# giuspugl/COSMOMAP2

Measured on AMD Instinct MI355X. Metric: TOD samples/s through P^T N^-1 P, higher is better.
Workload: dtype f64

## Files before the change

cosmomap2_amd/csrc/cm2_os_policy.h:

```cpp
#pragma once
#include <cstddef>
#include <cstdint>
#include <vector>

namespace cm2::os {

constexpr int kT = 256;
constexpr int kPts = 32;
constexpr int kHalo = 2048;
constexpr int N = kT * kPts;
constexpr int W = 2 * N;
constexpr int HOP = W - 2 * kHalo;
constexpr int RR = 2;
constexpr int RSLOTS = (kPts - 8) / RR;
constexpr int RLEN = 512 * RSLOTS;
constexpr int NLIST = 2 + RR;
constexpr int PER = 2 * N + HOP;
constexpr int LDSD = N + N / 32;
constexpr int list_off(int l) { return l <= 2 ? l * N : 2 * N + (l - 2) * RLEN; }
constexpr int list_len(int l) { return l < 2 ? N : RLEN; }

struct WinDesc {
    int64_t start, len, lo, hi;
    int32_t blk, pad;
};

inline std::vector<WinDesc> windows(const std::vector<int64_t> &off)
{
    std::vector<WinDesc> wins;
    for (size_t b = 0; b + 1 < off.size(); ++b)
        for (int64_t s0 = off[b]; s0 < off[b + 1]; s0 += HOP)
            wins.push_back({s0, off[b + 1] - s0 < HOP ? off[b + 1] - s0 : HOP, off[b], off[b + 1], (int32_t)b, 0});
    return wins;
}

inline int rmax(int64_t ntiles)
{
    const int64_t bound = ntiles > 0 && ntiles < N ? ntiles : N;
    return (int)((bound + 63) / 64 * 64);
}

constexpr int kTabRows = 8;
inline bool table_fits(int rmax_) { return rmax_ <= kTabRows * kT; }

enum class Builder { sorted, direct, inverse };
struct ListChoice { Builder builder; int mode, rmax; };
inline ListChoice choose_lists(int want_lists, bool build_sort, bool has_tile_off, int64_t ntiles)
{
    const int want = want_lists ? want_lists : (ntiles >= 768 ? 3 : 2);
    const bool direct = !build_sort && has_tile_off && ntiles > 0 && ntiles <= 4096;
    const int r = rmax(ntiles);
    const Builder b = !direct ? Builder::sorted : (want == 3 && table_fits(r) ? Builder::inverse : Builder::direct);
    return {b, b == Builder::inverse ? 3 : (want >= 2 && table_fits(r) ? 2 : 1), r};
}

inline uint32_t descriptor_bytes(int64_t nvalid, bool flat)
{
    return nvalid > 0 && nvalid * 8 < (int64_t)0xFFFFFFF0u && !flat ? (uint32_t)(nvalid * 8) : 0u;
}

inline size_t kernel_lds_bytes(int mode, int rmax_)
{
    return sizeof(double) * (size_t)LDSD + (mode >= 2 ? sizeof(uint32_t) * 2 * (size_t)rmax_ : 0) + 2048;
}

}
```

cosmomap2_amd/csrc/cm2_overlap_save.hip:

```cpp
#include "cm2_os_lists.h"

#include <cstring>
#include <memory>
#include <mutex>

using namespace cm2;

namespace {

constexpr double kCos32[32] = {1.0, 0.9807852804032304, 0.9238795325112867, 0.8314696123025452, 0.7071067811865476, 0.5555702330196022, 0.3826834323650898, 0.19509032201612828, 0.0, -0.19509032201612828, -0.3826834323650898, -0.5555702330196022, -0.7071067811865476, -0.8314696123025452, -0.9238795325112867, -0.9807852804032304, -1.0, -0.9807852804032304, -0.9238795325112867, -0.8314696123025452, -0.7071067811865476, -0.5555702330196022, -0.3826834323650898, -0.19509032201612828, 0.0, 0.19509032201612828, 0.3826834323650898, 0.5555702330196022, 0.7071067811865476, 0.8314696123025452, 0.9238795325112867, 0.9807852804032304};
constexpr double kSin32[32] = {0.0, 0.19509032201612828, 0.3826834323650898, 0.5555702330196022, 0.7071067811865476, 0.8314696123025452, 0.9238795325112867, 0.9807852804032304, 1.0, 0.9807852804032304, 0.9238795325112867, 0.8314696123025452, 0.7071067811865476, 0.5555702330196022, 0.3826834323650898, 0.19509032201612828, 0.0, -0.19509032201612828, -0.3826834323650898, -0.5555702330196022, -0.7071067811865476, -0.8314696123025452, -0.9238795325112867, -0.9807852804032304, -1.0, -0.9807852804032304, -0.9238795325112867, -0.8314696123025452, -0.7071067811865476, -0.5555702330196022, -0.3826834323650898, -0.19509032201612828};

__host__ __device__ constexpr int ilog2(int r) { return r <= 1 ? 0 : 1 + ilog2(r >> 1); }

template <int R>
__host__ __device__ constexpr int brev(int m)
{
    int out = 0;
    for (int b = 0; b < ilog2(R); ++b) out |= ((m >> b) & 1) << (ilog2(R) - 1 - b);
    return out;
}

template <class T> __device__ __forceinline__ T ld_list(const T *p) { return __builtin_nontemporal_load(p); }


#ifndef CM2_OS_TIMING
#define CM2_OS_TIMING 0
#endif
#if CM2_OS_TIMING & 1
#define OS_XF(...) do { } while (0)
#else
#define OS_XF(...) do { __VA_ARGS__; } while (0)
#endif

#ifdef CM2_OS_STAMPS
static unsigned long long *g_os_stamps_host = nullptr;
static unsigned long long *os_stamp_buf()
{
    static unsigned long long *dummy = nullptr;
    if (g_os_stamps_host) return g_os_stamps_host;
    if (!dummy && cm2::dev_malloc(&dummy, sizeof(unsigned long long) * 8 * (1 << 20)) != hipSuccess) abort();
    return dummy;
}
#define OS_STAMP_PARAM , unsigned long long *__restrict__ stamps
#define OS_STAMP_ARG , os_stamp_buf()
#define OS_STAMP(i) (stamps[(int64_t)win * 8 + (i)] = __builtin_amdgcn_s_memtime())
#else
#define OS_STAMP_PARAM
#define OS_STAMP_ARG
#define OS_STAMP(i) do { } while (0)
#endif

template <int L>
__device__ __forceinline__ int reg_base(int t)
{
    if (L == 1) return t + (t >> 5);
    if (L == 2) return (t >> 4) * 264 + (t & 15);
    return 33 * t;
}
template <int L>
__host__ __device__ constexpr int reg_off(int m)
{
    return L == 1 ? 264 * m : (L == 2 ? 4224 * (m >> 4) + 16 * (m & 15) + ((m & 15) >> 1) : m);
}
template <int PERM>
__host__ __device__ constexpr int reg_slot(int m)
{
    return PERM == 32 ? brev<32>(m) : (PERM == 16 ? 16 * (m >> 4) + brev<16>(m & 15) : m);
}

template <int FROM, int TO, int PERM>
__device__ __forceinline__ void reg_exchange(double (&a)[kPts], double *__restrict__ buf, int t)
{
    double *__restrict__ wp = buf + reg_base<FROM>(t);
    const double *__restrict__ rp = buf + reg_base<TO>(t);
#pragma unroll
    for (int m = 0; m < kPts; ++m) wp[reg_off<FROM>(m)] = a[reg_slot<PERM>(m)];
    __syncthreads();
#pragma unroll
    for (int m = 0; m < kPts; ++m) a[m] = rp[reg_off<TO>(m)];
    __syncthreads();
}

template <int R, int OFF>
__device__ __forceinline__ void dft_sub(double (&re)[kPts], double (&im)[kPts])
{
#pragma unroll
    for (int h = R / 2; h >= 1; h >>= 1) {
#pragma unroll
        for (int blk = 0; blk < R; blk += 2 * h) {
#pragma unroll
            for (int i = 0; i < h; ++i) {
                const int a = OFF + blk + i, b = a + h;
                const int tw = i * (32 / (2 * h));
                const double ar = re[a], ai = im[a], br = re[b], bi = im[b];
                re[a] = ar + br;
                im[a] = ai + bi;
                const double dr = ar - br, di = ai - bi;
                if (tw == 0) {
                    re[b] = dr;
                    im[b] = di;
                } else if (tw == 8) {
                    re[b] = di;
                    im[b] = -dr;
                } else {
                    const double c = kCos32[tw], s = kSin32[tw];
                    re[b] = dr * c + di * s;
                    im[b] = di * c - dr * s;
                }
            }
        }
    }
}

template <int R, int OFF>
__device__ __forceinline__ void dit_sub(double (&re)[kPts], double (&im)[kPts])
{
#pragma unroll
    for (int h = 1; h <= R / 2; h <<= 1) {
#pragma unroll
        for (int blk = 0; blk < R; blk += 2 * h) {
#pragma unroll
            for (int i = 0; i < h; ++i) {
                const int a = OFF + blk + i, b = a + h;
                const int tw = i * (32 / (2 * h));
                double tr, ti;
                if (tw == 0) {
                    tr = re[b];
                    ti = im[b];
                } else if (tw == 8) {
                    tr = im[b];
                    ti = -re[b];
                } else {
                    const double c = kCos32[tw], s = kSin32[tw];
                    tr = re[b] * c + im[b] * s;
                    ti = im[b] * c - re[b] * s;
                }
                const double ar = re[a], ai = im[a];
                re[a] = ar + tr;
                im[a] = ai + ti;
                re[b] = ar - tr;
                im[b] = ai - ti;
            }
        }
    }
}

template <int R, int OFF>
__device__ __forceinline__ void reg_fwd(double (&xr)[kPts], double (&xi)[kPts], double2 w1)
{
    dft_sub<R, OFF>(xr, xi);
    double cr = 1.0, ci = 0.0;
#pragma unroll
    for (int m = 1; m < R; ++m) {
        const double nr = cr * w1.x - ci * w1.y;
        ci = cr * w1.y + ci * w1.x;
        cr = nr;
        const int i = OFF + brev<R>(m);
        const double tr = xr[i] * cr - xi[i] * ci;
        xi[i] = xr[i] * ci + xi[i] * cr;
        xr[i] = tr;
    }
}

template <int R, int OFF>
__device__ __forceinline__ void reg_inv(double (&xr)[kPts], double (&xi)[kPts], double2 w1)
{
    double cr = 1.0, ci = 0.0;
#pragma unroll
    for (int m = 1; m < R; ++m) {
        const double nr = cr * w1.x - ci * w1.y;
        ci = cr * w1.y + ci * w1.x;
        cr = nr;
        const int i = OFF + m;
        const double tr = xr[i] * cr + xi[i] * ci;
        xi[i] = xi[i] * cr - xr[i] * ci;
        xr[i] = tr;
    }
    dft_sub<R, OFF>(xi, xr);
}

typedef unsigned int v2u_t __attribute__((ext_vector_type(2)));
template <int E>
__device__ __forceinline__ void q_request(const uint16_t *q, int t, uint32_t (&qq)[E / 2])
{
    asm volatile("" : "+v"(t));
    const v2u_t *p = reinterpret_cast<const v2u_t *>(q) + (E / 4) * 64 * (t >> 6) + (t & 63);
#pragma unroll
    for (int i = 0; i < E / 4; ++i) {
        const v2u_t v = __builtin_nontemporal_load(p + 64 * i);
        qq[2 * i] = v.x;
        qq[2 * i + 1] = v.y;
    }
}
template <int E2>
__device__ __forceinline__ uint32_t q_word(const uint32_t (&qq)[E2], int u) { return (qq[u >> 1] >> (16 * (u & 1))) & 0xFFFFu; }

struct ListArgs {
    const uint32_t *k;
    const uint16_t *q;
    const ListHdr *hdr;
    const uint32_t *tab;
};

__device__ __forceinline__ void tab_dma(const uint32_t *gtab, uint32_t *tab_lds, int rmax, int wave_, int t)
{
    int wave = wave_;
    asm volatile("" : "+s"(wave));
    asm volatile("" : "+v"(t));
    const uint32_t *g = gtab + 64 * wave + (t & 63);
#pragma unroll
    for (int i = 0; i < kTabRows; ++i)
        if (64 * wave + kT * i < rmax)
            __builtin_amdgcn_global_load_lds((const __attribute__((address_space(1))) void *)(g + kT * i),
                                             (__attribute__((address_space(3))) void *)(tab_lds + 64 * wave + kT * i),
                                             4, 0, 0);
}

template <int E, class F>
__device__ __forceinline__ void run_decode(F starts, const uint32_t *__restrict__ tab_lds, int wbase, uint32_t nvalid,
                                           uint32_t s0, uint32_t (&kk)[E])
{
    int rb = wbase;
    asm volatile("" : "+v"(s0));
#pragma unroll
    for (int u = 0; u < E; ++u) {
        const bool flag = starts(u);
        const uint64_t mask = __ballot(flag);
        const int below = __builtin_amdgcn_mbcnt_hi((uint32_t)(mask >> 32),
                                                    __builtin_amdgcn_mbcnt_lo((uint32_t)mask, 0u));
        int r = rb + below + (flag ? 1 : 0);
        rb += __popcll(mask);
        r = r < 0 ? 0 : r;
        const uint32_t s = s0 + 64u * (uint32_t)u;
        const uint32_t a = tab_lds[r] + s;
        kk[u] = s < nvalid ? a : kInvalidSample;
    }
}
template <int E>
__device__ __forceinline__ void rc_decode(const uint32_t (&qq)[E / 2], const uint32_t *__restrict__ tab_lds,
                                          int wbase, uint32_t nvalid, int t, uint32_t (&kk)[E])
{
    run_decode<E>([&](int u) { return (qq[u >> 1] & (0x8000u << (16 * (u & 1)))) != 0u; }, tab_lds, wbase, nvalid,
                  (uint32_t)slot_of<E>(t, 0), kk);
}


template <int E>
__device__ __forceinline__ void idecode(uint32_t fw, const uint32_t *__restrict__ tab_lds, int wbase,
                                        uint32_t nvalid, uint32_t soff, int t, uint32_t (&kk)[E])
{
    run_decode<E>([&](int u) { return ((fw >> u) & 1u) != 0u; }, tab_lds, wbase, nvalid,
                  soff + (uint32_t)slot_of<E>(t, 0), kk);
}

template <int BP>
__device__ __forceinline__ void partner_filter_half(double (&zr)[kPts], double (&zi)[kPts], double *__restrict__ buf,
                                                    double *__restrict__ xbuf, int t, const double2 *__restrict__ ab_own,
                                                    const double2 *__restrict__ ab_blk)
{
    constexpr int H = kPts / 2;
    double *__restrict__ wp = buf + reg_base<3>(t);
    const bool special = t < 8;
    const double2 *__restrict__ ab_prt = ab_blk + (special ? t : 263 - t);
    double2 ca[BP], cb[BP];
    auto request = [&](int m0) {
        int o = m0 * kT;
        asm volatile("" : "+v"(o));
#pragma unroll
        for (int i = 0; i < BP; ++i) {
            ca[i] = ab_own[o + i * kT];
            cb[i] = ab_prt[(kPts - 1) * kT - o - i * kT];
        }
    };
    request(0);
    __builtin_amdgcn_sched_barrier(0);
#pragma unroll
    for (int j = 0; j < H; ++j) {
        wp[H + j] = zr[reg_slot<16>(H + j)];
        wp[j] = zi[reg_slot<16>(H + j)];
    }
    if (special) {
#pragma unroll
        for (int j = 0; j < H; ++j) {
            xbuf[t * H + j] = zr[reg_slot<16>(j)];
            xbuf[(8 + t) * H + j] = zi[reg_slot<16>(j)];
        }
    }
    __syncthreads();
    if (!special) {
        double *__restrict__ pp = buf + 33 * (263 - t) + 31;
#pragma unroll
        for (int m0 = 0; m0 < H; m0 += BP) {
            if (m0 > 0) request(m0);
#pragma unroll
            for (int i0 = 0; i0 < BP; i0 += 4) {
                double pre[4], pim[4];
#pragma unroll
                for (int i = 0; i < 4; ++i) {
                    pre[i] = pp[-(m0 + i0 + i)];
                    pim[i] = pp[-H - (m0 + i0 + i)];
                }
#pragma unroll
                for (int i = 0; i < 4; ++i) {
                    const int m = m0 + i0 + i, sl = reg_slot<16>(m);
                    const double a = ca[i0 + i].x, b = ca[i0 + i].y, ap = cb[i0 + i].x, bp = cb[i0 + i].y;
                    const double nr = a * zr[sl] + b * pim[i];
                    const double ni = a * zi[sl] + b * pre[i];
                    const double qr = ap * pre[i] + bp * zi[sl];
                    const double qi = ap * pim[i] + bp * zr[sl];
                    zr[sl] = nr;
                    zi[sl] = ni;
                    pp[-m] = qr;
                    pp[-H - m] = qi;
                }
            }
            __builtin_amdgcn_sched_barrier(0);
        }
    } else {
        const int tl = t == 0 ? 0 : 8 - t;
        const double *__restrict__ up = buf + 33 * (7 - t) + 47;
#pragma unroll
        for (int m0 = 0; m0 < H; m0 += BP) {
            if (m0 > 0) request(m0);
#pragma unroll
            for (int i = 0; i < BP; ++i) {
                const int m = m0 + i, sl = reg_slot<16>(m);
                const int ms = t == 0 ? (m == 0 ? 0 : H - m) : H - 1 - m;
                const double pre_ = xbuf[tl * H + ms], pim_ = xbuf[(8 + tl) * H + ms];
                const double nr = ca[i].x * zr[sl] + ca[i].y * pim_;
                const double ni = ca[i].x * zi[sl] + ca[i].y * pre_;
                zr[sl] = nr;
                zi[sl] = ni;
                const int mu = kPts - 1 - m, su = reg_slot<16>(mu);
                const double ure = up[-mu], uim = up[-mu - H];
                zr[su] = cb[i].x * wp[mu] + cb[i].y * uim;
                zi[su] = cb[i].x * wp[mu - H] + cb[i].y * ure;
            }
            __builtin_amdgcn_sched_barrier(0);
        }
    }
    __syncthreads();
    if (!special) {
#pragma unroll
        for (int j = 0; j < H; ++j) {
            zr[reg_slot<16>(H + j)] = wp[H + j];
            zi[reg_slot<16>(H + j)] = wp[j];
        }
    }
    __syncthreads();
}

__device__ __forceinline__ void forward_passes(double (&zr)[kPts], double (&zi)[kPts], double *buf, int t,
                                               const double2 *Wtw)
{
    const double2 w_a = Wtw[t];
    const double2 w_b = Wtw[kPts * (t & 15)];
    reg_fwd<kPts, 0>(zr, zi, w_a);
    reg_exchange<1, 2, kPts>(zr, buf, t);
    reg_exchange<1, 2, kPts>(zi, buf, t);
    reg_fwd<16, 0>(zr, zi, w_b);
    reg_fwd<16, 16>(zr, zi, w_b);
    reg_exchange<2, 3, 16>(zr, buf, t);
    reg_exchange<2, 3, 16>(zi, buf, t);
}

__device__ __forceinline__ void inverse_tail(double (&zr)[kPts], double (&zi)[kPts], double *buf, int t, double2 w_bi,
                                             double2 w_ai)
{
    reg_inv<16, 0>(zr, zi, w_bi);
    reg_inv<16, 16>(zr, zi, w_bi);
    reg_exchange<2, 1, 16>(zr, buf, t);
    reg_exchange<2, 1, 16>(zi, buf, t);
    reg_inv<kPts, 0>(zr, zi, w_ai);
}

template <int MODE, bool BUF>
__global__ __launch_bounds__(kT, 2) void k_os_real(
    const WinDesc *__restrict__ wins, int nwin, const double2 *__restrict__ Wtw, const double2 *Wtw_inv,
    const double2 *__restrict__ AB, const uint32_t *__restrict__ lst_k, const uint16_t *__restrict__ lst_q,
    const ListHdr *__restrict__ hdrs, const uint32_t *__restrict__ tabs, int rmax, const double *__restrict__ v,
    double *__restrict__ out, uint32_t nbytes, const IListHdr *__restrict__ ihdrs,
    const uint32_t *__restrict__ iflags OS_STAMP_PARAM)
{
    constexpr int N = os::N, H = kPts / 2;
    constexpr int ER = os::RLEN / kT;
    __amdgpu_buffer_rsrc_t v_rs, o_rs;
    if constexpr (BUF) {
        v_rs = __builtin_amdgcn_make_buffer_rsrc(const_cast<double *>(v), 0, (int)nbytes, 0x00020000);
        o_rs = __builtin_amdgcn_make_buffer_rsrc(out, 0, (int)nbytes, 0x00020000);
    }
    auto gather = [&](uint32_t k) -> double {
        if constexpr (BUF) {
            const v2u_t r = __builtin_amdgcn_raw_buffer_load_b64(v_rs, k * 8u, 0, 0);
            return __builtin_bit_cast(double, r);
        } else {
            return v[k != kInvalidSample ? k : 0u];
        }
    };
    auto keep = [&](uint32_t k, double x) -> double {
        if constexpr (BUF) return x;
        return k != kInvalidSample ? x : 0.0;
    };
    extern __shared__ double buf[];
    uint32_t *__restrict__ tab_lds = reinterpret_cast<uint32_t *>(buf + os::LDSD);
    const int t = threadIdx.x;
    const int per_xcd = (nwin + 7) / 8;
    const int win = (blockIdx.x & 7) * per_xcd + (blockIdx.x >> 3);
    if (win >= nwin) return;
    const WinDesc wd = wins[win];
    const int64_t w0 = wd.start - kHalo;
    const int wave = __builtin_amdgcn_readfirstlane(t >> 6);
    OS_STAMP(0);

    auto list_args = [&](int l) {
        ListArgs la;
        const int64_t e0 = (int64_t)win * os::PER + os::list_off(l);
        la.k = nullptr, la.q = nullptr, la.hdr = nullptr, la.tab = nullptr;
        if constexpr (MODE == 1) la.k = lst_k + e0;
        if constexpr (MODE == 1 || MODE == 2) la.q = lst_q + e0;
        if constexpr (MODE == 2) {
            la.hdr = hdrs + ((int64_t)win * os::NLIST + l);
            la.tab = tabs + ((int64_t)win * os::NLIST + l) * rmax;
        }
        return la;
    };

    double zr[kPts], zi[kPts];
    if constexpr (MODE == 0) {
#pragma unroll
        for (int h = 0; h < 2; ++h) {
            double vv[kPts];
#pragma unroll
            for (int u = 0; u < kPts; ++u) {
                const int64_t ts = w0 + (int64_t)h * N + t + u * kT;
                vv[u] = (ts >= wd.lo && ts < wd.hi) ? v[ts] : 0.0;
            }
#pragma unroll
            for (int u = 0; u < kPts; ++u) buf[t + u * kT] = vv[u];
            __syncthreads();
            const double2 *__restrict__ sp = reinterpret_cast<const double2 *>(buf) + t;
#pragma unroll
            for (int m = 0; m < H; ++m) {
                const double2 p = sp[256 * m];
                zr[h * H + m] = p.x;
                zi[h * H + m] = p.y;
            }
            __syncthreads();
        }
    } else if constexpr (MODE == 3) {
        const IListHdr *__restrict__ h0 = ihdrs + (int64_t)win * 2;
        const uint32_t *__restrict__ pl = reinterpret_cast<const uint32_t *>(lst_q + (int64_t)win * os::PER);
        uint32_t fw[2], pp[kPts];
        tab_dma(tabs + ((int64_t)win * 2) * rmax, tab_lds, rmax, wave, t);
        fw[0] = iflags[((int64_t)win * 2) * 512 + t];
        fw[1] = iflags[((int64_t)win * 2) * 512 + 256 + t];
        const uint32_t nv = h0->nvalid;
        const int wb0 = h0->wbase[wave], wb1 = h0->wbase[4 + wave];
#pragma unroll
        for (int m = 0; m < kPts; ++m) pp[m] = pl[t + kT * m];
        __syncthreads();
        double va[kPts], vb[kPts];
        {
            uint32_t kk[kPts];
            idecode<kPts>(fw[0], tab_lds, wb0, nv, 0u, t, kk);
#pragma unroll
            for (int u = 0; u < kPts; ++u) va[u] = keep(kk[u], gather(kk[u]));
        }
        __builtin_amdgcn_sched_barrier(0);
        {
            uint32_t kk[kPts];
            idecode<kPts>(fw[1], tab_lds, wb1, nv, (uint32_t)N, t, kk);
#pragma unroll
            for (int u = 0; u < kPts; ++u) vb[u] = keep(kk[u], gather(kk[u]));
        }
        __builtin_amdgcn_sched_barrier(0);
#pragma unroll
        for (int j = 0; j < 2; ++j) {
#pragma unroll
            for (int u = 0; u < kPts; ++u) buf[slot_of<kPts>(t, u)] = j ? vb[u] : va[u];
            if (j == 1) {
                int tj = t;
                asm volatile("" : "+v"(tj));
#pragma unroll
                for (int m = 0; m < kPts; ++m) pp[m] = pl[tj + kT * m];
            }
            __syncthreads();
#pragma unroll
            for (int m = 0; m < kPts; ++m) {
                const uint32_t lo = (pp[m] & 0xFFFFu) - (uint32_t)(j * N), hi = (pp[m] >> 16) - (uint32_t)(j * N);
                const bool inl = lo < (uint32_t)N, inh = hi < (uint32_t)N;
                const double x = buf[inl ? lo : 0u], y = buf[inh ? hi : 0u];
                if (j == 0) {
                    zr[m] = inl ? x : 0.0;
                    zi[m] = inh ? y : 0.0;
                } else {
                    zr[m] = inl ? x : zr[m];
                    zi[m] = inh ? y : zi[m];
                }
            }
            __syncthreads();
        }
    } else {
        const ListArgs l0 = list_args(0), l1 = list_args(1);
        uint32_t qa[kPts / 2], qb[kPts / 2], ka[kPts], kb[kPts];
        uint32_t nva = 0, nvb = 0;
        int wba = -1, wbb = -1;
        if constexpr (MODE == 2) {
            nva = l0.hdr->nvalid;
            nvb = l1.hdr->nvalid;
            wba = l0.hdr->wbase[wave];
            wbb = l1.hdr->wbase[wave];
            tab_dma(l0.tab, tab_lds, rmax, wave, t);
            tab_dma(l1.tab, tab_lds + rmax, rmax, wave, t);
        }
        q_request<kPts>(l0.q, t, qa);
        if constexpr (MODE == 1) {
#pragma unroll
            for (int u = 0; u < kPts; ++u) ka[u] = ld_list(l0.k + slot_of<kPts>(t, u));
        }
        q_request<kPts>(l1.q, t, qb);
        if constexpr (MODE == 1) {
#pragma unroll
            for (int u = 0; u < kPts; ++u) kb[u] = ld_list(l1.k + slot_of<kPts>(t, u));
        }
        if constexpr (MODE == 2) {
            __syncthreads();
            OS_STAMP(6);
            rc_decode<kPts>(qa, tab_lds, wba, nva, t, ka);
        }
        __builtin_amdgcn_sched_barrier(0);
        double va[kPts], vv[kPts];
        if constexpr (MODE == 2) rc_decode<kPts>(qb, tab_lds + rmax, wbb, nvb, t, kb);
#pragma unroll
        for (int u = 0; u < kPts; ++u) va[u] = gather(ka[u]);
#pragma unroll
        for (int u = 0; u < kPts; ++u) vv[u] = gather(kb[u]);
        __builtin_amdgcn_sched_barrier(0);
#pragma unroll
        for (int u = 0; u < kPts; ++u) buf[q_word(qa, u) & 0x7FFFu] = keep(ka[u], va[u]);
        OS_STAMP(7);
        __syncthreads();
        const double2 *__restrict__ sp = reinterpret_cast<const double2 *>(buf) + t;
#pragma unroll
        for (int m = 0; m < H; ++m) {
            const double2 p = sp[256 * m];
            zr[m] = p.x;
            zi[m] = p.y;
        }
        __syncthreads();
#pragma unroll
        for (int u = 0; u < kPts; ++u) buf[q_word(qb, u) & 0x7FFFu] = keep(kb[u], vv[u]);
        __syncthreads();
#pragma unroll
        for (int m = 0; m < H; ++m) {
            const double2 p = sp[256 * m];
            zr[H + m] = p.x;
            zi[H + m] = p.y;
        }
        __syncthreads();
    }

    OS_STAMP(1);
    OS_XF(forward_passes(zr, zi, buf, t, Wtw));
    const double2 *ab = AB + (int64_t)wd.blk * N + t;
    OS_XF(dft_sub<16, 0>(zr, zi));
    OS_XF(dft_sub<16, 16>(zr, zi));
    OS_STAMP(2);
    OS_XF(partner_filter_half<(MODE == 1 && !BUF) ? 4 : 8>(zr, zi, buf, reinterpret_cast<double *>(tab_lds + 2 * rmax),
                                                           t, ab, AB + (int64_t)wd.blk * N));
    (void)ab;
    OS_STAMP(3);
    OS_XF(dit_sub<16, 0>(zi, zr));
    OS_XF(dit_sub<16, 16>(zi, zr));
    const double2 w_bi = Wtw_inv[kPts * (t & 15)], w_ai = Wtw_inv[t];
    OS_XF(reg_exchange<3, 2, 0>(zr, buf, t));
    OS_XF(reg_exchange<3, 2, 0>(zi, buf, t));
    asm volatile("" : : "v"(w_bi.x), "v"(w_bi.y), "v"(w_ai.x), "v"(w_ai.y));
    __builtin_amdgcn_sched_barrier(0);
    if constexpr (MODE == 3) {
        constexpr int NP = kPts - 8;
        int l1 = 1;
        asm volatile("" : "+s"(l1));
        const IListHdr *h1 = ihdrs + (int64_t)win * 2 + l1;
        const uint32_t *tg = tabs + ((int64_t)win * 2 + l1) * rmax;
        const uint32_t *fg = iflags + ((int64_t)win * 2 + l1) * 512 + t;
        const uint32_t nv1 = h1->nvalid;
        uint32_t fr[os::RR], rp[NP];
        const uint32_t *rl = reinterpret_cast<const uint32_t *>(lst_q + (int64_t)win * os::PER + 2 * N);
        tab_dma(tg, tab_lds + rmax, rmax, wave, t);
#pragma unroll
        for (int j = 0; j < os::RR; ++j) fr[j] = fg[256 * j];
        int t0 = t;
        asm volatile("" : "+v"(t0));
#pragma unroll
        for (int m = 0; m < NP; ++m) rp[m] = rl[t0 + kT * m];
        __builtin_amdgcn_sched_barrier(0);
        OS_XF(inverse_tail(zr, zi, buf, t, w_bi, w_ai));
        OS_STAMP(4);
#pragma unroll
        for (int j = 0; j < os::RR; ++j) {
            if (j > 0) {
                __syncthreads();
                int tj = t;
                asm volatile("" : "+v"(tj));
#pragma unroll
                for (int m = 0; m < NP; ++m) rp[m] = rl[tj + kT * m];
            }
#pragma unroll
            for (int m = 0; m < NP; ++m) {
                const uint32_t lo = (rp[m] & 0xFFFFu) - (uint32_t)(j * os::RLEN), hi = (rp[m] >> 16) - (uint32_t)(j * os::RLEN);
                buf[lo < (uint32_t)os::RLEN ? lo : (uint32_t)N] = zr[brev<kPts>(m + 4)];
                buf[hi < (uint32_t)os::RLEN ? hi : (uint32_t)N + 1u] = zi[brev<kPts>(m + 4)];
            }
            __syncthreads();
            uint32_t ks[ER];
            idecode<ER>(fr[j], tab_lds + rmax, h1->wbase[4 * j + wave], nv1, (uint32_t)(j * os::RLEN), t, ks);
            double rv[ER];
#pragma unroll
            for (int u = 0; u < ER; ++u) rv[u] = buf[slot_of<ER>(t, u)];
#pragma unroll
            for (int u = 0; u < ER; ++u) {
                if constexpr (BUF) {
                    __builtin_amdgcn_raw_buffer_store_b64(__builtin_bit_cast(v2u_t, rv[u]), o_rs, ks[u] * 8u, 0, 0);
                } else {
                    if (ks[u] != kInvalidSample) out[ks[u]] = rv[u];
                }
            }
        }
    } else {
        uint32_t qs[ER / 2], ks[ER];
        uint32_t nvs = 0;
        int wbs = -1;
        auto request_results = [&](int j, auto &qq, uint32_t &nv, int &wb, uint32_t *tdst) {
            if constexpr (MODE != 0) {
                int lj = 2 + j;
                asm volatile("" : "+s"(lj));
                const ListArgs ls = list_args(lj);
                if constexpr (MODE == 2) {
                    nv = ls.hdr->nvalid;
                    wb = ls.hdr->wbase[wave];
                    tab_dma(ls.tab, tdst, rmax, wave, t);
                }
                q_request<ER>(ls.q, t, qq);
            }
        };
        constexpr bool EARLY = MODE == 2 || (MODE == 1 && BUF);
        uint32_t qs1[ER / 2];
        uint32_t nv1 = 0;
        int wb1 = -1;
        request_results(0, qs, nvs, wbs, tab_lds);
        __builtin_amdgcn_sched_barrier(0);
        OS_XF(inverse_tail(zr, zi, buf, t, w_bi, w_ai));
        OS_STAMP(4);
#pragma unroll
        for (int j = 0; j < os::RR; ++j) {
            const uint32_t *tabj = tab_lds + (EARLY && j > 0 ? rmax : 0);
            if (j > 0) {
                __syncthreads();
                if constexpr (EARLY) {
#pragma unroll
                    for (int i = 0; i < ER / 2; ++i) qs[i] = qs1[i];
                    nvs = nv1;
                    wbs = wb1;
                } else {
                    request_results(j, qs, nvs, wbs, tab_lds);
                    if constexpr (MODE == 2) __syncthreads();
                }
            }
            if constexpr (MODE == 2) rc_decode<ER>(qs, tabj, wbs, nvs, t, ks);
            double2 *__restrict__ sp = reinterpret_cast<double2 *>(buf) + t;
#pragma unroll
            for (int mm = 0; mm < os::RSLOTS; ++mm) {
                const int m = 4 + j * os::RSLOTS + mm;
                sp[256 * mm] = make_double2(zr[brev<kPts>(m)], zi[brev<kPts>(m)]);
            }
            if constexpr (MODE == 1) {
                const ListArgs ls = list_args(2 + j);
#pragma unroll
                for (int u = 0; u < ER; ++u) ks[u] = ld_list(ls.k + slot_of<ER>(t, u));
            }
            __syncthreads();
            if constexpr (EARLY)
                if (j + 1 < os::RR) request_results(j + 1, qs1, nv1, wb1, tab_lds + rmax);
            if constexpr (MODE == 0) {
#pragma unroll
                for (int u = 0; u < ER; ++u) {
                    const int e = t + u * kT;
                    const int64_t o = (int64_t)j * os::RLEN + e;
                    if (o < wd.len) out[wd.start + o] = buf[e];
                }
            } else {
                double rv[ER];
#pragma unroll
                for (int u = 0; u < ER; ++u) rv[u] = buf[q_word(qs, u) & 0x7FFFu];
#pragma unroll
                for (int u = 0; u < ER; ++u) {
                    if constexpr (BUF) {
                        __builtin_amdgcn_raw_buffer_store_b64(__builtin_bit_cast(v2u_t, rv[u]), o_rs, ks[u] * 8u, 0, 0);
                    } else {
                        if (ks[u] != kInvalidSample) out[ks[u]] = rv[u];
                    }
                }
            }
        }
    }
    OS_STAMP(5);
}

__global__ void k_real_twiddles(int N, double2 *__restrict__ W)
{
    const int t = blockIdx.x * blockDim.x + threadIdx.x;
    if (t < N) W[t] = make_double2(cospi(2.0 * t / N), -sinpi(2.0 * t / N));
}

__global__ void k_real_cos_table(int N, double *__restrict__ ct)
{
    const int m = blockIdx.x * blockDim.x + threadIdx.x;
    if (m <= N) ct[m] = cospi((double)m / (double)N);
}

constexpr int kSpecK = 1024;
__global__ __launch_bounds__(256) void k_real_spectrum(int nb, int64_t lambda, int N,
                                                        const double *__restrict__ bands,
                                                        const double *__restrict__ ct_g,
                                                        double *__restrict__ Hs)
{
    extern __shared__ double ct[];
    constexpr int PER = kSpecK / 256;
    const int chunks = (N + 1 + kSpecK - 1) / kSpecK;
    const int b = blockIdx.x / chunks, c = blockIdx.x % chunks;
    for (int m = threadIdx.x; m <= N; m += 256) ct[m] = ct_g[m];
    __syncthreads();
    const double *band = bands + (int64_t)b * lambda;
    const int mask = 2 * N - 1;
    int k[PER], m[PER];
    double acc[PER];
#pragma unroll
    for (int u = 0; u < PER; ++u) {
        k[u] = c * kSpecK + u * 256 + (int)threadIdx.x;
        m[u] = (int)(((lambda - 1) * (int64_t)k[u]) & mask);
        acc[u] = 0.0;
    }
    for (int64_t j = lambda - 1; j >= 1; --j) {
        const double a = band[j];
#pragma unroll
        for (int u = 0; u < PER; ++u) {
            const int f = m[u] <= N ? m[u] : 2 * N - m[u];
            acc[u] += a * ct[f];
            m[u] = (m[u] - k[u]) & mask;
        }
    }
#pragma unroll
    for (int u = 0; u < PER; ++u)
        if (k[u] <= N) Hs[(int64_t)b * (N + 1) + k[u]] = band[0] + 2.0 * acc[u];
}

__global__ __launch_bounds__(256) void k_real_alpha_beta(int nb, const double *__restrict__ Hs, double2 *__restrict__ AB)
{
    constexpr int N = os::N;
    const int64_t total = (int64_t)nb * N;
    const int64_t stride = (int64_t)gridDim.x * blockDim.x;
    for (int64_t e = (int64_t)blockIdx.x * blockDim.x + threadIdx.x; e < total; e += stride) {
        const int64_t b = e / N;
        const int a = (int)(e - b * N);
        const int d1 = a / 256, d2 = (a / 16) % 16, d3 = a % 16;
        const int k = d1 + kPts * d2 + 16 * kPts * d3;
        const double *h = Hs + b * (N + 1);
        const double hk = h[k], hp = h[N - k];
        const double S = 0.5 * (hk + hp), Dd = 0.5 * (hk - hp);
        const double th = (double)k / (double)N;
        const int t = a / kPts, m = a % kPts;
        AB[b * N + (int64_t)m * kT + t] = make_double2((S - Dd * sinpi(th)) / (double)N,
                                                        (Dd * cospi(th)) / (double)N);
    }
}

}

namespace cm2 {

constexpr size_t kListCache = 3;

struct FusedOS {
    int64_t nwin = 0;
    WinDesc *d_wins = nullptr;
    double2 *d_AB = nullptr;
    double2 *d_W = nullptr;
    int want_lists = 0;
    bool build_sort = false;
    bool flat = false;
    int64_t sort_chunk_windows = 0;
    std::mutex mu;
    std::vector<std::shared_ptr<OsLists>> cache;
};

void fused_os_destroy(FusedOS *f)
{
    if (!f) return;
    f->cache.clear();
    void *ptrs[] = {f->d_wins, f->d_AB, f->d_W};
    for (void *q : ptrs)
        if (q) (void)cm2::dev_free(q);
    delete f;
}

bool fused_os_supported(int64_t lambda) { return lambda >= 1 && lambda - 1 <= kHalo; }

int64_t fused_os_length(const FusedOS *f) { return f ? os::N : 0; }

int fused_os_create(FusedOS **out, const double *d_bands, int64_t lambda, const std::vector<int64_t> &off,
                    hipStream_t stream)
{
    CM2_CHECK(out != nullptr, "fused_os_create: out is NULL");
    *out = nullptr;
    CM2_CHECK(fused_os_supported(lambda), "fused overlap-save supports lambda <= 2049, got %lld",
              (long long)lambda);
    FusedOS *f = new FusedOS();
    struct Guard { FusedOS *f; ~Guard() { if (f) fused_os_destroy(f); } } guard{f};
    if (const char *e = getenv("CM2_OS_LISTS")) {
        if (!strcmp(e, "plain")) f->want_lists = 1;
        else if (!strcmp(e, "rc")) f->want_lists = 2;
        else if (!strcmp(e, "inv")) f->want_lists = 3;
    }
    if (const char *e = getenv("CM2_OS_LIST_BUILD")) f->build_sort = strcmp(e, "sort") == 0;
    f->flat = getenv("CM2_OS_FLAT") != nullptr;
    if (const char *e = getenv("CM2_OS_LIST_CHUNK_PAIRS")) f->sort_chunk_windows = atoll(e);
    const int64_t nb = (int64_t)off.size() - 1;
    const std::vector<WinDesc> wins = os::windows(off);
    f->nwin = (int64_t)wins.size();
    CM2_CHECK(f->nwin * 4 < ((int64_t)1 << 31), "fused overlap-save: too many windows (%lld)", (long long)f->nwin);
    CM2_HIP(cm2::dev_malloc(&f->d_wins, sizeof(WinDesc) * (wins.size() ? wins.size() : 1)));
    if (!wins.empty())
        CM2_HIP(cm2::upload(f->d_wins, wins.data(), sizeof(WinDesc) * wins.size(), nullptr));
    CM2_HIP(cm2::dev_malloc(&f->d_AB, sizeof(double2) * (nb > 0 ? nb : 1) * os::N));
    if (nb > 0) {
        DevTemp<double> Hs;
        CM2_HIP(Hs.alloc(nb * (os::N + 1)));
        DevTemp<double> ct;
        CM2_HIP(ct.alloc(os::N + 1));
        k_real_cos_table<<<(os::N + 256) / 256, 256, 0, stream>>>(os::N, ct);
        CM2_LAUNCH_OK();
        const size_t ct_lds = sizeof(double) * (os::N + 1);
        static size_t ct_granted[64] = {0};
        CM2_HIP(ensure_dynamic_lds((const void *)k_real_spectrum, ct_lds, ct_granted));
        const int chunks = (os::N + 1 + kSpecK - 1) / kSpecK;
        k_real_spectrum<<<(int)nb * chunks, 256, ct_lds, stream>>>((int)nb, lambda, os::N, d_bands, ct, Hs);
        CM2_LAUNCH_OK();
        k_real_alpha_beta<<<grid_for(nb * os::N), kBlock, 0, stream>>>((int)nb, Hs, f->d_AB);
        CM2_LAUNCH_OK();
        CM2_HIP(hipStreamSynchronize(stream));
    }
    CM2_HIP(cm2::dev_malloc(&f->d_W, sizeof(double2) * os::N));
    k_real_twiddles<<<(os::N + 255) / 256, 256, 0, stream>>>(os::N, f->d_W);
    CM2_LAUNCH_OK();
    CM2_HIP(hipStreamSynchronize(stream));
    guard.f = nullptr;
    *out = f;
    return 0;
}

template <int MODE, bool BUF>
static int os_launch_t(const FusedOS *f, const OsLists *ls, const double *d_v, double *d_out, uint32_t nbytes,
                       hipStream_t stream)
{
    const int rmax = ls ? ls->rmax : 0;
    const size_t lds = os::kernel_lds_bytes(MODE, rmax);
    static size_t granted[64] = {0};
    CM2_HIP(ensure_dynamic_lds((const void *)k_os_real<MODE, BUF>, lds, granted));
    if (f->nwin == 0) return 0;
    const int grid = (int)(((f->nwin + 7) / 8) * 8);
    k_os_real<MODE, BUF><<<grid, kT, lds, stream>>>(
        f->d_wins, (int)f->nwin, f->d_W, f->d_W, f->d_AB, ls ? ls->d_lst_k : nullptr, ls ? ls->d_lst_q : nullptr,
        ls ? ls->d_hdrs : nullptr, ls ? ls->d_tabs : nullptr, rmax, d_v, d_out, nbytes, ls ? ls->d_ihdrs : nullptr,
        ls ? ls->d_iflags : nullptr OS_STAMP_ARG);
    CM2_LAUNCH_OK();
    return 0;
}

static int os_launch(const FusedOS *f, const OsLists *ls, int64_t nvalid, const double *d_v, double *d_out,
                     hipStream_t stream)
{
    if (f->nwin == 0) return 0;
    const uint32_t nbytes = os::descriptor_bytes(nvalid, f->flat);
    static constexpr decltype(&os_launch_t<1, false>) launch[3][2] = {{os_launch_t<1, false>, os_launch_t<1, true>},
                                                                      {os_launch_t<2, false>, os_launch_t<2, true>},
                                                                      {os_launch_t<3, false>, os_launch_t<3, true>}};
    if (ls->mode == 1 || ((ls->mode == 2 || ls->mode == 3) && os::table_fits(ls->rmax)))
        return launch[ls->mode - 1][nbytes != 0u](f, ls, d_v, d_out, nbytes, stream);
    set_error("fused overlap-save: run table of %d words per list does not fit the kernel", ls->rmax);
    return CM2_ERR_ARGUMENT;
}

int fused_os_apply(const FusedOS *f, const double *d_v, double *d_out, hipStream_t stream)
{
    return os_launch_t<0, false>(f, nullptr, d_v, d_out, 0, stream);
}

static int os_lists_for(FusedOS *f, const OsPlanView &pv, hipStream_t stream, std::shared_ptr<OsLists> *out)
{
    std::lock_guard<std::mutex> lock(f->mu);
    for (size_t i = 0; i < f->cache.size(); ++i)
        if (f->cache[i]->plan_id == pv.plan_id) {
            std::shared_ptr<OsLists> hit = f->cache[i];
            f->cache.erase(f->cache.begin() + (long)i);
            f->cache.insert(f->cache.begin(), hit);
            *out = hit;
            return 0;
        }
    const os::ListChoice c = os::choose_lists(f->want_lists, f->build_sort, pv.d_tile_off != nullptr, pv.ntiles);
    std::shared_ptr<OsLists> ls = std::make_shared<OsLists>();
    ls->plan_id = pv.plan_id;
    CM2_CHECK(f->nwin * os::NLIST < ((int64_t)1 << 31), "fused overlap-save: too many lists (%lld)",
              (long long)(f->nwin * os::NLIST));
    if (f->nwin == 0) {
        ls->mode = 1;
    } else if (int rc = os_build_lists(c, f->d_wins, f->nwin, ls.get(), pv, f->sort_chunk_windows, stream)) {
        return rc;
    }
    f->cache.insert(f->cache.begin(), ls);
    while (f->cache.size() > kListCache) f->cache.pop_back();
    *out = ls;
    return 0;
}

int fused_os_prepare_indexed(FusedOS *f, const OsPlanView &pv, hipStream_t stream)
{
    std::shared_ptr<OsLists> ls;
    return os_lists_for(f, pv, stream, &ls);
}

int fused_os_apply_indexed(FusedOS *f, const OsPlanView &pv, const double *d_v, double *d_out, hipStream_t stream)
{
    std::shared_ptr<OsLists> ls;
    if (int rc = os_lists_for(f, pv, stream, &ls)) return rc;
    return os_launch(f, ls.get(), pv.nvalid, d_v, d_out, stream);
}

double fused_os_tile_info(const FusedOS *f_, int *kernel)
{
    FusedOS *f = const_cast<FusedOS *>(f_);
    std::shared_ptr<OsLists> ls;
    if (f) {
        std::lock_guard<std::mutex> lock(f->mu);
        if (!f->cache.empty()) ls = f->cache.front();
    }
    if (kernel) {
        kernel[0] = f ? os::kPts : 0;
        kernel[1] = ls ? ls->mode : 0;
    }
    if (!f) return 0.0;
    const double hop = (double)os::HOP, win = (double)os::W;
    const double lists = ls && ls->bytes_per_window > 0 ? ls->bytes_per_window : 6.0 * (win + hop);
    return (lists + 8.0 * win + 8.0 * hop) / hop;
}

#ifdef CM2_OS_STAMPS
extern "C" int cm2_os_debug_stamps(unsigned long long *d_buf)
{
    g_os_stamps_host = d_buf;
    return 0;
}
#endif

}
```

Before: 71.75 billion.

## Store half-spectrum S/D filter coefficients and rebuild twiddle factors on the fly

Replaces the precomputed per-bin alpha/beta table (N double2 per block, own plus partner loads) with a half-size S/D table plus a small per-thread twiddle seed. The seed is rotated by constant 32-point angles in registers to rebuild the coefficients, and partner coefficients for the special threads come through LDS. Coefficient loads are also software-pipelined one batch ahead. This cuts global coefficient traffic and load count in the filter stage, at the cost of extra FMAs, registers and a small LDS slot. It also adds static asserts on LDS occupancy.

```diff
diff --git a/cosmomap2_amd/csrc/cm2_os_policy.h b/cosmomap2_amd/csrc/cm2_os_policy.h
--- a/cosmomap2_amd/csrc/cm2_os_policy.h
+++ b/cosmomap2_amd/csrc/cm2_os_policy.h
@@ -17,6 +17,7 @@
 constexpr int NLIST = 2 + RR;
 constexpr int PER = 2 * N + HOP;
 constexpr int LDSD = N + N / 32;
+constexpr int SDREC = N / 2 + 8 * (kPts / 2);
 constexpr int list_off(int l) { return l <= 2 ? l * N : 2 * N + (l - 2) * RLEN; }
 constexpr int list_len(int l) { return l < 2 ? N : RLEN; }
 
@@ -59,9 +60,16 @@
     return nvalid > 0 && nvalid * 8 < (int64_t)0xFFFFFFF0u && !flat ? (uint32_t)(nvalid * 8) : 0u;
 }
 
-inline size_t kernel_lds_bytes(int mode, int rmax_)
+constexpr size_t kernel_lds_bytes(int mode, int rmax_)
 {
     return sizeof(double) * (size_t)LDSD + (mode >= 2 ? sizeof(uint32_t) * 2 * (size_t)rmax_ : 0) + 2048;
 }
 
+constexpr size_t kLdsPerCU = 160 * 1024;
+constexpr int kTwoPerCuRmax = 1536;
+constexpr int workgroups_per_cu(int mode, int rmax_) { return 2 * kernel_lds_bytes(mode, rmax_) <= kLdsPerCU ? 2 : 1; }
+static_assert(workgroups_per_cu(0, 0) == 2 && workgroups_per_cu(1, kTabRows * kT) == 2, "time order and plain lists");
+static_assert(workgroups_per_cu(2, kTwoPerCuRmax) == 2 && workgroups_per_cu(3, kTwoPerCuRmax) == 2 &&
+              workgroups_per_cu(3, kTwoPerCuRmax + 64) == 1, "k_os_real: two workgroups per CU up to 1536 table words");
+
 }
diff --git a/cosmomap2_amd/csrc/cm2_overlap_save.hip b/cosmomap2_amd/csrc/cm2_overlap_save.hip
--- a/cosmomap2_amd/csrc/cm2_overlap_save.hip
+++ b/cosmomap2_amd/csrc/cm2_overlap_save.hip
@@ -254,32 +254,49 @@
                   soff + (uint32_t)slot_of<E>(t, 0), kk);
 }
 
+__device__ __forceinline__ double2 unit_turn(double2 e, int M)
+{
+    if (M == 0) return e;
+    if (M == 8) return make_double2(-e.y, e.x);
+    return make_double2(e.x * kCos32[M] - e.y * kSin32[M], e.y * kCos32[M] + e.x * kSin32[M]);
+}
+constexpr double kCosPi256 = 0.9999247018391445, kSinPi256 = 0.012271538285719925;
+
 template <int BP>
 __device__ __forceinline__ void partner_filter_half(double (&zr)[kPts], double (&zi)[kPts], double *__restrict__ buf,
-                                                    double *__restrict__ xbuf, int t, const double2 *__restrict__ ab_own,
-                                                    const double2 *__restrict__ ab_blk)
+                                                    double *__restrict__ xbuf, int t, const double2 *__restrict__ sd_own,
+                                                    const double *__restrict__ sd_up, const double2 *__restrict__ e_tab)
 {
     constexpr int H = kPts / 2;
     double *__restrict__ wp = buf + reg_base<3>(t);
     const bool special = t < 8;
-    const double2 *__restrict__ ab_prt = ab_blk + (special ? t : 263 - t);
-    double2 ca[BP], cb[BP];
-    auto request = [&](int m0) {
+    double2 sd[BP], sn[BP];
+    auto request = [&](int m0, double2 (&dst)[BP]) {
         int o = m0 * kT;
         asm volatile("" : "+v"(o));
 #pragma unroll
-        for (int i = 0; i < BP; ++i) {
-            ca[i] = ab_own[o + i * kT];
-            cb[i] = ab_prt[(kPts - 1) * kT - o - i * kT];
-        }
+        for (int i = 0; i < BP; ++i) dst[i] = sd_own[o + i * kT];
     };
-    request(0);
+    request(0, sd);
     __builtin_amdgcn_sched_barrier(0);
-#pragma unroll
-    for (int j = 0; j < H; ++j) {
+    constexpr int PRE = 2;
+#pragma unroll
+    for (int j = 0; j < PRE; ++j) {
         wp[H + j] = zr[reg_slot<16>(H + j)];
         wp[j] = zi[reg_slot<16>(H + j)];
     }
+    __builtin_amdgcn_sched_barrier(0);
+    int tt = t;
+    asm volatile("" : "+v"(tt));
+    const double up_word = sd_up[tt];
+    const double2 e0 = e_tab[tt];
+    __builtin_amdgcn_sched_barrier(0);
+#pragma unroll
+    for (int j = PRE; j < H; ++j) {
+        wp[H + j] = zr[reg_slot<16>(H + j)];
+        wp[j] = zi[reg_slot<16>(H + j)];
+    }
+    wp[kPts] = up_word;
     if (special) {
 #pragma unroll
         for (int j = 0; j < H; ++j) {
@@ -292,7 +309,8 @@
         double *__restrict__ pp = buf + 33 * (263 - t) + 31;
 #pragma unroll
         for (int m0 = 0; m0 < H; m0 += BP) {
-            if (m0 > 0) request(m0);
+            if (m0 + BP < H) request(m0 + BP, sn);
+            __builtin_amdgcn_sched_barrier(0);
 #pragma unroll
             for (int i0 = 0; i0 < BP; i0 += 4) {
                 double pre[4], pim[4];
@@ -304,38 +322,56 @@
 #pragma unroll
                 for (int i = 0; i < 4; ++i) {
                     const int m = m0 + i0 + i, sl = reg_slot<16>(m);
-                    const double a = ca[i0 + i].x, b = ca[i0 + i].y, ap = cb[i0 + i].x, bp = cb[i0 + i].y;
+                    const double2 e = unit_turn(e0, m);
+                    const double S = sd[i0 + i].x, D = sd[i0 + i].y;
+                    const double ds = D * e.y, b = D * e.x, a = S - ds, ap = S + ds;
                     const double nr = a * zr[sl] + b * pim[i];
                     const double ni = a * zi[sl] + b * pre[i];
-                    const double qr = ap * pre[i] + bp * zi[sl];
-                    const double qi = ap * pim[i] + bp * zr[sl];
+                    const double qr = ap * pre[i] + b * zi[sl];
+                    const double qi = ap * pim[i] + b * zr[sl];
                     zr[sl] = nr;
                     zi[sl] = ni;
                     pp[-m] = qr;
                     pp[-H - m] = qi;
                 }
             }
+            if (m0 + BP < H) {
+#pragma unroll
+                for (int i = 0; i < BP; ++i) sd[i] = sn[i];
+            }
             __builtin_amdgcn_sched_barrier(0);
         }
     } else {
         const int tl = t == 0 ? 0 : 8 - t;
         const double *__restrict__ up = buf + 33 * (7 - t) + 47;
+        const double *__restrict__ ur = buf + 33 * t + kPts;
+        const double2 e1 = make_double2(e0.x * kCosPi256 - e0.y * kSinPi256, e0.y * kCosPi256 + e0.x * kSinPi256);
 #pragma unroll
         for (int m0 = 0; m0 < H; m0 += BP) {
-            if (m0 > 0) request(m0);
+            if (m0 + BP < H) request(m0 + BP, sn);
+            __builtin_amdgcn_sched_barrier(0);
 #pragma unroll
             for (int i = 0; i < BP; ++i) {
                 const int m = m0 + i, sl = reg_slot<16>(m);
                 const int ms = t == 0 ? (m == 0 ? 0 : H - m) : H - 1 - m;
                 const double pre_ = xbuf[tl * H + ms], pim_ = xbuf[(8 + tl) * H + ms];
-                const double nr = ca[i].x * zr[sl] + ca[i].y * pim_;
-                const double ni = ca[i].x * zi[sl] + ca[i].y * pre_;
+                const double2 e = unit_turn(e0, m);
+                const double a = sd[i].x - sd[i].y * e.y, b = sd[i].y * e.x;
+                const double nr = a * zr[sl] + b * pim_;
+                const double ni = a * zi[sl] + b * pre_;
                 zr[sl] = nr;
                 zi[sl] = ni;
                 const int mu = kPts - 1 - m, su = reg_slot<16>(mu);
                 const double ure = up[-mu], uim = up[-mu - H];
-                zr[su] = cb[i].x * wp[mu] + cb[i].y * uim;
-                zi[su] = cb[i].x * wp[mu - H] + cb[i].y * ure;
+                const double2 eu = unit_turn(e1, H - 1 - m);
+                const double Su = ur[33 * 8 * m], Du = ur[33 * (128 + 8 * m)];
+                const double au = Su - Du * eu.y, bu = Du * eu.x;
+                zr[su] = au * wp[mu] + bu * uim;
+                zi[su] = au * wp[mu - H] + bu * ure;
+            }
+            if (m0 + BP < H) {
+#pragma unroll
+                for (int i = 0; i < BP; ++i) sd[i] = sn[i];
             }
             __builtin_amdgcn_sched_barrier(0);
         }
@@ -378,7 +414,7 @@
 template <int MODE, bool BUF>
 __global__ __launch_bounds__(kT, 2) void k_os_real(
     const WinDesc *__restrict__ wins, int nwin, const double2 *__restrict__ Wtw, const double2 *Wtw_inv,
-    const double2 *__restrict__ AB, const uint32_t *__restrict__ lst_k, const uint16_t *__restrict__ lst_q,
+    const double2 *__restrict__ SD, const uint32_t *__restrict__ lst_k, const uint16_t *__restrict__ lst_q,
     const ListHdr *__restrict__ hdrs, const uint32_t *__restrict__ tabs, int rmax, const double *__restrict__ v,
     double *__restrict__ out, uint32_t nbytes, const IListHdr *__restrict__ ihdrs,
     const uint32_t *__restrict__ iflags OS_STAMP_PARAM)
@@ -563,13 +599,14 @@
 
     OS_STAMP(1);
     OS_XF(forward_passes(zr, zi, buf, t, Wtw));
-    const double2 *ab = AB + (int64_t)wd.blk * N + t;
+    const double2 *sd = SD + (int64_t)wd.blk * os::SDREC + t;
     OS_XF(dft_sub<16, 0>(zr, zi));
     OS_XF(dft_sub<16, 16>(zr, zi));
     OS_STAMP(2);
-    OS_XF(partner_filter_half<(MODE == 1 && !BUF) ? 4 : 8>(zr, zi, buf, reinterpret_cast<double *>(tab_lds + 2 * rmax),
-                                                           t, ab, AB + (int64_t)wd.blk * N));
-    (void)ab;
+    OS_XF(partner_filter_half<(MODE == 1 && !BUF) ? 4 : 8>(
+        zr, zi, buf, reinterpret_cast<double *>(tab_lds + 2 * rmax), t, sd,
+        reinterpret_cast<const double *>(SD + (int64_t)wd.blk * os::SDREC + N / 2), Wtw_inv + N));
+    (void)sd;
     OS_STAMP(3);
     OS_XF(dit_sub<16, 0>(zi, zr));
     OS_XF(dit_sub<16, 16>(zi, zr));
@@ -711,7 +748,12 @@
 __global__ void k_real_twiddles(int N, double2 *__restrict__ W)
 {
     const int t = blockIdx.x * blockDim.x + threadIdx.x;
-    if (t < N) W[t] = make_double2(cospi(2.0 * t / N), -sinpi(2.0 * t / N));
+    if (t < N) {
+        W[t] = make_double2(cospi(2.0 * t / N), -sinpi(2.0 * t / N));
+    } else if (t < N + kT) {
+        const int k0 = ((t - N) >> 3) + 64 * ((t - N) & 7);
+        W[t] = make_double2(cospi((double)k0 / N), sinpi((double)k0 / N));
+    }
 }
 
 __global__ void k_real_cos_table(int N, double *__restrict__ ct)
@@ -756,23 +798,32 @@
         if (k[u] <= N) Hs[(int64_t)b * (N + 1) + k[u]] = band[0] + 2.0 * acc[u];
 }
 
-__global__ __launch_bounds__(256) void k_real_alpha_beta(int nb, const double *__restrict__ Hs, double2 *__restrict__ AB)
-{
-    constexpr int N = os::N;
-    const int64_t total = (int64_t)nb * N;
+__global__ __launch_bounds__(256) void k_real_sd(int nb, const double *__restrict__ Hs, double2 *__restrict__ SD)
+{
+    constexpr int N = os::N, R = os::SDREC, UP = 8 * (kPts / 2);
+    const int64_t total = (int64_t)nb * (N / 2 + UP);
     const int64_t stride = (int64_t)gridDim.x * blockDim.x;
     for (int64_t e = (int64_t)blockIdx.x * blockDim.x + threadIdx.x; e < total; e += stride) {
-        const int64_t b = e / N;
-        const int a = (int)(e - b * N);
-        const int d1 = a / 256, d2 = (a / 16) % 16, d3 = a % 16;
-        const int k = d1 + kPts * d2 + 16 * kPts * d3;
+        const int64_t b = e / (N / 2 + UP);
+        const int a = (int)(e - b * (N / 2 + UP));
         const double *h = Hs + b * (N + 1);
+        int k;
+        if (a < N / 2) {
+            const int m = a / kT, t = a % kT;
+            k = (t >> 3) + 64 * (t & 7) + 512 * m;
+        } else {
+            const int m = (a - N / 2) / 8, t = (a - N / 2) % 8;
+            k = 64 * t + 32 + 512 * (kPts / 2 - 1 - m);
+        }
         const double hk = h[k], hp = h[N - k];
-        const double S = 0.5 * (hk + hp), Dd = 0.5 * (hk - hp);
-        const double th = (double)k / (double)N;
-        const int t = a / kPts, m = a % kPts;
-        AB[b * N + (int64_t)m * kT + t] = make_double2((S - Dd * sinpi(th)) / (double)N,
-                                                        (Dd * cospi(th)) / (double)N);
+        const double S = 0.5 * (hk + hp) / (double)N, Dd = 0.5 * (hk - hp) / (double)N;
+        if (a < N / 2) {
+            SD[b * R + a] = make_double2(S, Dd);
+        } else {
+            double *up = reinterpret_cast<double *>(SD + b * R + N / 2);
+            up[a - N / 2] = S;
+            up[UP + a - N / 2] = Dd;
+        }
     }
 }
 
@@ -785,7 +836,7 @@
 struct FusedOS {
     int64_t nwin = 0;
     WinDesc *d_wins = nullptr;
-    double2 *d_AB = nullptr;
+    double2 *d_SD = nullptr;
     double2 *d_W = nullptr;
     int want_lists = 0;
     bool build_sort = false;
@@ -799,7 +850,7 @@
 {
     if (!f) return;
     f->cache.clear();
-    void *ptrs[] = {f->d_wins, f->d_AB, f->d_W};
+    void *ptrs[] = {f->d_wins, f->d_SD, f->d_W};
     for (void *q : ptrs)
         if (q) (void)cm2::dev_free(q);
     delete f;
@@ -833,7 +884,7 @@
     CM2_HIP(cm2::dev_malloc(&f->d_wins, sizeof(WinDesc) * (wins.size() ? wins.size() : 1)));
     if (!wins.empty())
         CM2_HIP(cm2::upload(f->d_wins, wins.data(), sizeof(WinDesc) * wins.size(), nullptr));
-    CM2_HIP(cm2::dev_malloc(&f->d_AB, sizeof(double2) * (nb > 0 ? nb : 1) * os::N));
+    CM2_HIP(cm2::dev_malloc(&f->d_SD, sizeof(double2) * (nb > 0 ? nb : 1) * os::SDREC));
     if (nb > 0) {
         DevTemp<double> Hs;
         CM2_HIP(Hs.alloc(nb * (os::N + 1)));
@@ -847,12 +898,12 @@
         const int chunks = (os::N + 1 + kSpecK - 1) / kSpecK;
         k_real_spectrum<<<(int)nb * chunks, 256, ct_lds, stream>>>((int)nb, lambda, os::N, d_bands, ct, Hs);
         CM2_LAUNCH_OK();
-        k_real_alpha_beta<<<grid_for(nb * os::N), kBlock, 0, stream>>>((int)nb, Hs, f->d_AB);
+        k_real_sd<<<grid_for(nb * os::SDREC), kBlock, 0, stream>>>((int)nb, Hs, f->d_SD);
         CM2_LAUNCH_OK();
         CM2_HIP(hipStreamSynchronize(stream));
     }
-    CM2_HIP(cm2::dev_malloc(&f->d_W, sizeof(double2) * os::N));
-    k_real_twiddles<<<(os::N + 255) / 256, 256, 0, stream>>>(os::N, f->d_W);
+    CM2_HIP(cm2::dev_malloc(&f->d_W, sizeof(double2) * (os::N + os::kT)));
+    k_real_twiddles<<<(os::N + os::kT + 255) / 256, 256, 0, stream>>>(os::N, f->d_W);
     CM2_LAUNCH_OK();
     CM2_HIP(hipStreamSynchronize(stream));
     guard.f = nullptr;
@@ -871,7 +922,7 @@
     if (f->nwin == 0) return 0;
     const int grid = (int)(((f->nwin + 7) / 8) * 8);
     k_os_real<MODE, BUF><<<grid, kT, lds, stream>>>(
-        f->d_wins, (int)f->nwin, f->d_W, f->d_W, f->d_AB, ls ? ls->d_lst_k : nullptr, ls ? ls->d_lst_q : nullptr,
+        f->d_wins, (int)f->nwin, f->d_W, f->d_W, f->d_SD, ls ? ls->d_lst_k : nullptr, ls ? ls->d_lst_q : nullptr,
         ls ? ls->d_hdrs : nullptr, ls ? ls->d_tabs : nullptr, rmax, d_v, d_out, nbytes, ls ? ls->d_ihdrs : nullptr,
         ls ? ls->d_iflags : nullptr OS_STAMP_ARG);
     CM2_LAUNCH_OK();
```

Measured after the change: 72.43 billion, median of 6. About the same (+0.9%).
